# ActiveVisionLab/nope-nerf

Hardware: AMD Instinct MI355X
Metric: training rays/sec (higher is better)
Workload: dtype f32; 1 GPU; BASELINE configs[1]: 1024 rays/GPU x 192 samples, D=256, fp32 via three fp16 MFMA terms per product (fwd, dgrad, wgrad 4x4 + encoding tiles); fp32_products=split2, adam_arithmetic=single, rays_per_gpu=1024, total_rays=1024, n_samples=192, hidden=256, parallelism=dp1 (ray-sharded, one flat all-reduce)

## Files before the change

### nope-nerf_amd/csrc/nnr_api.cpp

```cpp
#include <hip/hip_runtime.h>

#include <algorithm>
#include <cmath>
#include <cstdint>
#include <cstdlib>
#include <cstring>
#include <array>
#include <vector>

#include "../../include/nnr.h"
#include "nnr_device.h"
#include "nnr_kernels.h"
#include "nnr_layout.h"

using namespace nnr;

namespace {

thread_local int g_last_hip = 0;

int hip_fail(hipError_t e) {
    g_last_hip = (int)e;
    return NNR_E_HIP;
}

bool aligned16(const void* p) { return (reinterpret_cast<uintptr_t>(p) & 15u) == 0; }

int check_cfg(const nnr_cfg* c) {
    if (!c || c->n_rays <= 0 || c->n_samples <= 0) return NNR_E_BADCFG;
    if (c->hidden != 128 && c->hidden != 256) return NNR_E_UNSUPPORTED;
    if ((c->flags & NNR_F_TRAIN) && c->n_samples > 1024) return NNR_E_UNSUPPORTED;
    return NNR_OK;
}

WsLayout ws_layout(const nnr_cfg* c) {
    WsLayout w;
    w.S = (int64_t)c->n_rays * c->n_samples;
    w.S_pad = (w.S + kBlockSamples - 1) / kBlockSamples * kBlockSamples;
    w.D = c->hidden;
    w.train = (c->flags & NNR_F_TRAIN) != 0;
    w.bf16 = w.train && (c->flags & NNR_F_BF16) != 0;
    w.tile32 = w.train && (c->flags & (NNR_F_BF16 | NNR_F_SPLIT3)) == NNR_F_SPLIT3;
    return w;
}

int64_t plane(const WsLayout& w, int id) {
    int pitch;
    return w.plane(id, &pitch);
}

size_t packed_floats(int D, int mode) {
    if (mode == 3) return D == 256 ? (size_t)Layout<256, 3>::packed_floats : (size_t)Layout<128, 3>::packed_floats;
    if (mode == 2) return D == 256 ? (size_t)Layout<256, 2>::packed_floats : (size_t)Layout<128, 2>::packed_floats;
    if (mode == 1) return D == 256 ? (size_t)Layout<256, 1>::packed_floats : (size_t)Layout<128, 1>::packed_floats;
    return D == 256 ? (size_t)Layout<256>::packed_floats : (size_t)Layout<128>::packed_floats;
}
bool is_bf16(const nnr_cfg* c) { return (c->flags & NNR_F_BF16) != 0; }
bool is_split3(const nnr_cfg* c) { return (c->flags & (NNR_F_BF16 | NNR_F_SPLIT3)) == NNR_F_SPLIT3; }
bool is_split2(const nnr_cfg* c) { return is_split3(c) && (c->flags & NNR_F_SPLIT2) != 0; }
int weight_mode(const nnr_cfg* c) { return is_bf16(c) ? 1 : (is_split2(c) ? 3 : (is_split3(c) ? 2 : 0)); }

int chunks_per_ray(const nnr_cfg* c) {
    static const bool off = std::getenv("NNR_FLAT_GRID") != nullptr;
    const int unit = is_bf16(c) ? kBf16Tiles * kChunk : kChunk;
    const int waves = is_bf16(c) ? kBf16Waves : kWavesPerBlock;
    return (!off && c->n_samples % unit == 0 && c->n_rays % waves == 0) ? c->n_samples / unit : 0;
}

struct Unit {
    WgradJob j;
    int group;
};

std::vector<Unit> wgrad_units(int D) {
    std::vector<Unit> u;
    const int nb = D / 128;
    int group = 0;
    auto add = [&](int layer, int MI, int NI, int dpl, int dcol, int dvalid, int xpl, int xcol, int xvalid, int row0, int wcol0,
                   int rows_real, int cols_real, int ldw, int bias) {
        Unit x{};
        x.j = WgradJob{layer, MI, NI, dpl, dcol, dvalid, xpl, xcol, xvalid, row0, wcol0, rows_real, cols_real, ldw, 0, 0, bias, 0, -1, 0};
        x.group = group;
        u.push_back(x);
    };
    auto dxd = [&](int layer, int dpl, int xpl, int ldw, int cols_real) {
        for (int a = 0; a < nb; ++a)
            for (int b = 0; b < nb; ++b)
                add(layer, 4, 4, dpl, 128 * a, D - 128 * a, xpl, 128 * b, D - 128 * b, 128 * a, 128 * b, D, cols_real, ldw,
                    nb == 2 ? 2 + b : 1);
        ++group;
// ... 118 lines not shown
    const int64_t group_cost = 4 * 16 * 1000;
    const int64_t group_equiv = std::max<int64_t>(1, (cost_a + cost_b + group_cost / 2) / group_cost);
    const int n_blocks = (int)std::max<int64_t>(2, std::min<int64_t>(max_blocks, granules * group_equiv / kMinGranulesPerBlock));
    int nb_b = (int)((cost_b * n_blocks + (cost_a + cost_b) / 2) / (cost_a + cost_b));
    nb_b = groups.empty() ? n_blocks : std::max(1, std::min(n_blocks - 1, nb_b));
    const int nb_a = n_blocks - nb_b;

    std::vector<std::vector<WgradJob>> per_wave((size_t)n_blocks * 4);
    auto emit = [&](int wave, int unit, int64_t g0, int64_t g1) {
        if (g1 <= g0) return;
        WgradJob j = units[unit].j;
        j.k0 = (int32_t)(g0 * kGranule);
        j.k1 = (int32_t)(g1 * kGranule);
        j.split = unit;
        per_wave[wave].push_back(j);
    };
    const int64_t tape_a = granules * (int64_t)groups.size();
    for (int b = 0; b < nb_a; ++b) {
        const int64_t a0 = tape_a * b / nb_a, a1 = tape_a * (b + 1) / nb_a;
        for (int64_t g = a0 / granules; g <= (a1 - 1) / granules && a1 > a0; ++g) {
            const int64_t lo = std::max(a0, g * granules) - g * granules, hi = std::min(a1, (g + 1) * granules) - g * granules;
            for (int t = 0; t < 4; ++t) emit(4 * b + t, groups[g][t], lo, hi);
        }
    }
    static const bool coop = std::getenv("NNR_WGRAD_NO_COOP") == nullptr;
    if (split && coop)
        for (int wv = 0; wv < 4 * nb_a; ++wv)
            for (auto& j : per_wave[wv]) j.reserved = 1;
    if (!bundles.empty()) {
        int64_t tape = 0;
        for (int64_t cb : bundle_cost) tape += cb * granules;
        int64_t off = 0;
        for (size_t i = 0; i < bundles.size(); ++i) {
            const int64_t cb = bundle_cost[i], end = off + cb * granules;
            auto to_granule = [&](int64_t x) { return std::min(granules, std::max<int64_t>(0, (x - off + cb / 2) / cb)); };
            for (int b = 0; b < nb_b; ++b) {
                const int64_t c0 = tape * b / nb_b, c1 = tape * (b + 1) / nb_b;
                if (c1 <= off || c0 >= end) continue;
                const int64_t g0 = c0 <= off ? 0 : to_granule(c0), g1 = c1 >= end ? granules : to_granule(c1);
                for (int t = 0; t < 4; ++t)
                    for (int u : bundles[i][t]) emit(4 * (nb_a + b) + t, u, g0, g1);
            }
            off = end;
        }
    }
    const int nw_b = nb_b * 4;
    const int64_t tape_b = cost_b * granules;
    std::vector<int64_t> cuts((size_t)nw_b + 1);
    for (int v = 0; v <= nw_b; ++v) cuts[v] = tape_b * v / nw_b;
    int64_t off = 0;
    for (int u : bundles.empty() ? small : std::vector<int>{}) {
        const int64_t cu = weight(units[u].j), end = off + cu * granules;
        auto to_granule = [&](int64_t x) { return std::min(granules, std::max<int64_t>(0, (x - off + cu / 2) / cu)); };
        for (int v = 0; v < nw_b; ++v) {
            if (cuts[v + 1] <= off || cuts[v] >= end) continue;
            const int64_t g0 = cuts[v] <= off ? 0 : to_granule(cuts[v]);
            const int64_t g1 = cuts[v + 1] >= end ? granules : to_granule(cuts[v + 1]);
            emit(4 * nb_a + v, u, g0, g1);
        }
        off = end;
    }
    for (auto& v : per_wave)
        for (auto& j : v)
            if (is_enc2(j)) j.reserved = 2;
    Plan p;
    p.wave_first.push_back(0);
    for (auto& v : per_wave) {
        for (auto& j : v) p.jobs.push_back(j);
        p.wave_first.push_back((int32_t)p.jobs.size());
    }
    std::vector<std::vector<int>> by_tile(units.size());
    for (size_t i = 0; i < p.jobs.size(); ++i) by_tile[p.jobs[i].split].push_back((int)i);
    for (auto& v : by_tile) {
        std::sort(v.begin(), v.end(), [&](int x, int y) { return p.jobs[x].k0 < p.jobs[y].k0; });
        for (size_t s = 0; s < v.size(); ++s) {
            p.jobs[v[s]].split = (int32_t)s;
            p.jobs[v[s]].next_split = s + 1 < v.size() ? v[s + 1] : -1;
        }
        if (!v.empty()) p.heads.push_back(v[0]);
    }
    return p;
}

constexpr int32_t kPlanMagic = 0x4e4e5235;
size_t plan_bytes(const Plan& p) { return p.jobs.size() * sizeof(WgradJob) + (p.wave_first.size() + 1 + p.heads.size() + 4) * sizeof(int32_t); }

struct BUnit {
    int d_plane, d_g0, d_groups, x_plane, x_g0, x_groups, MT, NT, WR, WC, bias;
    int x2_plane = -1, x2_groups = 0;
};
struct BPlan {
    std::vector<WgradJobB> jobs;
    std::vector<int32_t> block_first;
    std::vector<WgradOutB> outs;
};

void bf16_units(int D, std::vector<BUnit>& units, std::vector<WgradOutB>& outs) {
    const int G = D / 16, Gh = D / 32;
    const bool big = D == 256;
    static const bool no_merge = std::getenv("NNR_WGRAD_NO_MERGE") != nullptr;
    const bool merge = big && !no_merge;
    auto out = [&](int unit, int layer, int d_row, int n_rows, int w_row, int x_col, int n_cols, int w_col, int ldw, int bias) {
        const BUnit& u = units[unit];
        outs.push_back(WgradOutB{unit, layer, d_row, n_rows, w_row, x_col, n_cols, w_col, ldw, bias, -1, u.MT, u.NT, u.WR, u.WC, 0});
    };
    auto dxd = [&](int layer, int dpl, int xpl, int ldw) {
        units.push_back(BUnit{dpl, 0, G, xpl, 0, G, big ? 4 : 2, big ? 4 : 2, 2, 2, 1});
        out((int)units.size() - 1, layer, 0, D, 0, 0, D, 0, ldw, 1);
    };
    auto dxe = [&](int layer, int dpl, int w_col, int ldw, int bias) {
        units.push_back(BUnit{dpl, 0, G, P_XE16, 0, kPosPad / 16, big ? 2 : 1, 2, 4, 1, bias});
        out((int)units.size() - 1, layer, 0, D, 0, 0, kPosReal, w_col, ldw, bias);
    };
    dxe(0, P_DH1 + 0, 0, kPosReal, 1);
    dxd(1, P_DH1 + 1, P_XH1 + 0, D);
    dxd(2, P_DH1 + 2, P_XH1 + 1, D);
    dxd(3, P_DH1 + 3, P_XH1 + 2, D);
    if (merge) {
        units.push_back(BUnit{P_DH1 + 4, 0, G, P_XH1 + 3, 0, G, 4, 5, 2, 2, 1, P_XE16, kPosPad / 16});
        out((int)units.size() - 1, 4, 0, D, 0, 0, D, 0, D + kPosReal, 1);
        out((int)units.size() - 1, 4, 0, D, 0, D, kPosReal, D, D + kPosReal, 0);
    } else {
        dxd(4, P_DH1 + 4, P_XH1 + 3, D + kPosReal);
        dxe(4, P_DH1 + 4, D, D + kPosReal, 0);
    }
    dxd(5, P_DH1 + 5, P_XH1 + 4, D);
    dxd(6, P_DH1 + 6, P_XH1 + 5, D);
    dxd(7, P_DH1 + 7, P_XH1 + 6, D);
    if (merge) {
        units.push_back(BUnit{P_DG, 0, Gh + 1, P_XH1 + 7, 0, G, 5, 3, 1, 3, 1, P_XF16, kDirPad / 16});
        out((int)units.size() - 1, kMergedLayer, 0, D / 2, 0, 0, D, 0, D, 1);
        out((int)units.size() - 1, 8, D / 2 + 3, 1, 0, 0, D, 0, D, 1);
        out((int)units.size() - 1, 10, 0, D / 2, 0, D, kDirReal, D, D + kDirReal, 0);
    } else {
        units.push_back(BUnit{P_DG, 0, Gh + 1, P_XH1 + 7, 0, G, big ? 5 : 3, big ? 2 : 1, 1, 4, 1});
        out((int)units.size() - 1, kMergedLayer, 0, D / 2, 0, 0, D, 0, D, 1);
        out((int)units.size() - 1, 8, D / 2 + 3, 1, 0, 0, D, 0, D, 1);
        units.push_back(BUnit{P_DG, 0, Gh, P_XF16, 0, kDirPad / 16, 1, 1, big ? 4 : 2, 1, 0});
        out((int)units.size() - 1, 10, 0, D / 2, 0, 0, kDirReal, D, D + kDirReal, 0);
    }
    units.push_back(BUnit{P_DG, Gh, 1, P_XG, 0, Gh, 1, 1, 1, big ? 4 : 2, 1});
    out((int)units.size() - 1, 11, 0, 3, 0, 0, D / 2, 0, D / 2, 1);
}

constexpr int64_t kMinTapePerBlock = 16 * 32;

BPlan build_plan_bf16(const nnr_cfg* c) {
    const WsLayout w = ws_layout(c);
    BPlan p;
    std::vector<BUnit> units;
    bf16_units(c->hidden, units, p.outs);
    const int64_t chunks = w.S_pad / 32;
    std::vector<int64_t> cost(units.size()), start(units.size() + 1, 0);
    for (size_t u = 0; u < units.size(); ++u) {
        cost[u] = units[u].d_groups + units[u].x_groups + units[u].x2_groups;
        start[u + 1] = start[u] + cost[u] * chunks;
    }
    const int64_t tape = start[units.size()];
    static const int max_blocks = [] {
        const char* e = std::getenv("NNR_WGRAD_MAX_BLOCKS");
        return e ? std::max(1, std::atoi(e)) : kMaxBlocks;
    }();
    const int n_blocks = (int)std::max<int64_t>(1, std::min<int64_t>(max_blocks, tape / kMinTapePerBlock));
    auto cut_chunk = [&](size_t u, int64_t x) {
        if (x <= start[u]) return (int64_t)0;
        if (x >= start[u + 1]) return chunks;
// ... 129 lines not shown
    int pitch = 0;
    const int64_t o = ws_layout(cfg).plane(pl, &pitch);
    if (pitch_out) *pitch_out = pitch;
    return pl < 0 ? -1 : o;
}

int nnr_ws_plane_layout(const nnr_cfg* cfg, int pl) {
    if (check_cfg(cfg) != NNR_OK) return -1;
    const WsLayout w = ws_layout(cfg);
    int pitch = 0;
    if (pl < 0 || w.plane(pl, &pitch) < 0) return -1;
    if (w.tiled(pl)) return 2;
    if (w.bf16 && ((pl >= P_XH1 && pl < P_XH1 + 8) || pl == P_XG || pl == P_XE16 || pl == P_XF16 || (pl >= P_DH1 && pl < P_DH1 + 8) || pl == P_DG)) return 1;
    return 0;
}

size_t nnr_plan_bytes(const nnr_cfg* cfg) {
    if (check_cfg(cfg) != NNR_OK) return 0;
    if (is_bf16(cfg)) return plan_bytes(build_plan_bf16(cfg));
    return plan_bytes(build_plan(cfg));
}

int nnr_plan_counts(const nnr_cfg* cfg, int32_t* n_jobs, int32_t* n_waves) {
    int rc = check_cfg(cfg);
    if (rc != NNR_OK) return rc;
    if (is_bf16(cfg)) {
        const BPlan p = build_plan_bf16(cfg);
        if (n_jobs) *n_jobs = (int32_t)p.jobs.size();
        if (n_waves) *n_waves = 4 * ((int32_t)p.block_first.size() - 1);
        return NNR_OK;
    }
    const Plan p = build_plan(cfg);
    if (n_jobs) *n_jobs = (int32_t)p.jobs.size();
    if (n_waves) *n_waves = (int32_t)p.wave_first.size() - 1;
    return NNR_OK;
}

int nnr_plan_build(const nnr_cfg* cfg, void* plan_host) {
    int rc = check_cfg(cfg);
    if (rc != NNR_OK) return rc;
    if (!plan_host) return NNR_E_BADCFG;
    if (is_bf16(cfg)) {
        const BPlan p = build_plan_bf16(cfg);
        char* out = static_cast<char*>(plan_host);
        std::memcpy(out, p.jobs.data(), p.jobs.size() * sizeof(WgradJobB));
        out += p.jobs.size() * sizeof(WgradJobB);
        std::memcpy(out, p.block_first.data(), p.block_first.size() * sizeof(int32_t));
        out += p.block_first.size() * sizeof(int32_t);
        std::memcpy(out, p.outs.data(), p.outs.size() * sizeof(WgradOutB));
        return NNR_OK;
    }
    const Plan p = build_plan(cfg);
    std::memcpy(plan_host, p.jobs.data(), p.jobs.size() * sizeof(WgradJob));
    char* tail = static_cast<char*>(plan_host) + p.jobs.size() * sizeof(WgradJob);
    std::memcpy(tail, p.wave_first.data(), p.wave_first.size() * sizeof(int32_t));
    tail += p.wave_first.size() * sizeof(int32_t);
    const int32_t n_heads = (int32_t)p.heads.size();
    std::memcpy(tail, &n_heads, sizeof(int32_t));
    std::memcpy(tail + sizeof(int32_t), p.heads.data(), p.heads.size() * sizeof(int32_t));
    const int32_t trailer[4] = {kPlanMagic, (int32_t)p.jobs.size(), (int32_t)p.wave_first.size() - 1, n_heads};
    std::memcpy(tail + sizeof(int32_t) * (1 + p.heads.size()), trailer, sizeof(trailer));
    return NNR_OK;
}

int nnr_pack_weights(const nnr_cfg* cfg, const nnr_params* p, float* packed, void* stream) {
    int rc = check_cfg(cfg);
    if (rc != NNR_OK) return rc;
    if (!p || !packed) return NNR_E_BADCFG;
    if (!aligned16(packed)) return NNR_E_ALIGN;
    PackArgs a;
    for (int i = 0; i < 12; ++i) {
        if (!p->weight[i] || !p->bias[i]) return NNR_E_BADCFG;
        a.w[i] = p->weight[i];
        a.b[i] = p->bias[i];
    }
    a.packed = packed;
    hipError_t e = launch_pack(cfg->hidden, a, weight_mode(cfg), (hipStream_t)stream);
    return e == hipSuccess ? NNR_OK : hip_fail(e);
}

static float* plane_max_of(const nnr_cfg* cfg, float* ws) {
    const WsLayout w = ws_layout(cfg);
    const size_t merged = (size_t)(cfg->hidden / 2) * cfg->hidden + cfg->hidden / 2;
    return ws + (size_t)w.total() + build_plan(cfg).jobs.size() * (size_t)kSlotFloats + merged;
}

static int mlp_fwd_impl(const nnr_cfg* cfg, const float* pts_o, const float* pts_d, const float* view_d, const float* z_lo,
                        const float* z_hi, const float* jitter, const float* packed, float* ws, float* fuse_rgb, float* fuse_dist,
                        void* stream) {
    int rc = check_cfg(cfg);
    if (rc != NNR_OK) return rc;
    if (!pts_o || !pts_d || !view_d || !z_lo || !z_hi || !packed || !ws) return NNR_E_BADCFG;
    if (!aligned16(packed) || !aligned16(ws)) return NNR_E_ALIGN;
    const WsLayout w = ws_layout(cfg);
    MlpFwdArgs a{};
    a.pts_o = pts_o; a.pts_d = pts_d; a.view_d = view_d; a.z_lo = z_lo; a.z_hi = z_hi; a.jitter = jitter;
    a.packed = packed;
    a.ws_out4 = ws + plane(w, P_OUT4);
    a.ws_z = ws + plane(w, P_Z);
    if (w.train) {
        a.ws_xe = ws + plane(w, P_XE);
        a.ws_xh = ws + plane(w, P_XH1);
        a.ws_xf = ws + plane(w, P_XF);
        a.ws_xg = ws + plane(w, P_XG);
        if (w.bf16) {
            a.ws_xe16 = ws + plane(w, P_XE16);
            a.ws_xf16 = ws + plane(w, P_XF16);
            a.ws_pts = ws + plane(w, P_DPTS);
            a.ws_view = ws + plane(w, P_DVIEW);
        }
        a.ws_mask = reinterpret_cast<uint32_t*>(ws + plane(w, P_MASK));
        if (is_split2(cfg)) {
            a.plane_max = plane_max_of(cfg, ws);
            hipError_t em = hipMemsetAsync(a.plane_max, 0, kPlaneMaxFloats * sizeof(float), (hipStream_t)stream);
            if (em != hipSuccess) return hip_fail(em);
        }
    }
    a.S = w.S; a.S_pad = w.S_pad; a.N = cfg->n_samples;
    a.chunks_per_ray = chunks_per_ray(cfg);
    a.fuse_rgb = fuse_rgb; a.fuse_dist = fuse_dist; a.flags = cfg->flags;
    hipError_t e = is_bf16(cfg) ? launch_mlp_fwd_bf16(cfg->hidden, a, w.train, (hipStream_t)stream)
                                : launch_mlp_fwd(cfg->hidden, a, w.train, (hipStream_t)stream, weight_mode(cfg));
    return e == hipSuccess ? NNR_OK : hip_fail(e);
}

int nnr_mlp_fwd(const nnr_cfg* cfg, const float* pts_o, const float* pts_d, const float* view_d, const float* z_lo,
                const float* z_hi, const float* jitter, const float* packed, float* ws, void* stream) {
    return mlp_fwd_impl(cfg, pts_o, pts_d, view_d, z_lo, z_hi, jitter, packed, ws, nullptr, nullptr, stream);
}

int nnr_composite_fwd(const nnr_cfg* cfg, float* rgb, float* dist, float* opt_alpha, float* opt_z, float* ws, void* stream) {
    int rc = check_cfg(cfg);
    if (rc != NNR_OK) return rc;
    if (!rgb || !dist || !ws) return NNR_E_BADCFG;
    const WsLayout w = ws_layout(cfg);
    CompositeArgs a{};
    a.ws_out4 = ws + plane(w, P_OUT4);
    a.ws_z = ws + plane(w, P_Z);
    a.rgb = rgb; a.dist = dist; a.opt_alpha = opt_alpha; a.opt_z = opt_z;
    a.R = cfg->n_rays; a.N = cfg->n_samples; a.flags = cfg->flags;
    hipError_t e = launch_composite_fwd(a, (hipStream_t)stream);
    return e == hipSuccess ? NNR_OK : hip_fail(e);
}

int nnr_render_fwd(const nnr_cfg* cfg, const float* pts_o, const float* pts_d, const float* view_d, const float* z_lo,
                   const float* z_hi, const float* jitter, const float* packed, float* rgb, float* dist, float* opt_alpha,
                   float* opt_z, float* ws, void* stream) {
    static const bool no_fuse = std::getenv("NNR_NO_FUSED_COMPOSITE") != nullptr;
    if (cfg && !(cfg->flags & NNR_F_TRAIN) && !opt_alpha && !opt_z && rgb && dist && !no_fuse && chunks_per_ray(cfg) > 0)
        return mlp_fwd_impl(cfg, pts_o, pts_d, view_d, z_lo, z_hi, jitter, packed, ws, rgb, dist, stream);
    int rc = nnr_mlp_fwd(cfg, pts_o, pts_d, view_d, z_lo, z_hi, jitter, packed, ws, stream);
    if (rc != NNR_OK) return rc;
    return nnr_composite_fwd(cfg, rgb, dist, opt_alpha, opt_z, ws, stream);
}

int nnr_ray_march(const nnr_cfg* cfg, const float* ray_o, const float* ray_d, float radius, const float* t_table, int32_t n_secant,
                  const float* packed, float* state, float* d_out, void* stream) {
    if (!cfg || cfg->n_rays <= 0 || n_secant < 0) return NNR_E_BADCFG;
    if (cfg->hidden != 128 && cfg->hidden != 256) return NNR_E_UNSUPPORTED;
    if (cfg->n_samples < 2 || cfg->n_samples > 1024 || (cfg->flags & (NNR_F_TRAIN | NNR_F_WHITE_BG)) || !is_split2(cfg)) return NNR_E_UNSUPPORTED;
    if (!ray_o || !ray_d || !t_table || !packed || !state || !d_out) return NNR_E_BADCFG;
    if (!aligned16(packed) || !aligned16(state)) return NNR_E_ALIGN;
    MarchArgs a{};
    a.ray_o = ray_o; a.ray_d = ray_d; a.t = t_table; a.packed = packed; a.state = state;
    a.radius = radius; a.R = cfg->n_rays; a.n_steps = cfg->n_samples;
    a.flags = cfg->flags & (NNR_F_RELU_SIGMA | NNR_F_DIST_ALPHA);
    const hipStream_t st = (hipStream_t)stream;
// ... 59 lines not shown

int nnr_composite_bwd(const nnr_cfg* cfg, const float* d_rgb, const float* d_dist, float* ws, void* stream) {
    int rc = check_cfg(cfg);
    if (rc != NNR_OK) return rc;
    if (!(cfg->flags & NNR_F_TRAIN) || !d_rgb || !d_dist || !ws) return NNR_E_BADCFG;
    const WsLayout w = ws_layout(cfg);
    CompositeArgs a{};
    a.ws_out4 = ws + plane(w, P_OUT4);
    a.ws_z = ws + plane(w, P_Z);
    a.ws_dout4 = ws + plane(w, P_DOUT4);
    a.d_rgb = d_rgb; a.d_dist = d_dist;
    a.R = cfg->n_rays; a.N = cfg->n_samples; a.flags = cfg->flags;
    hipError_t e = launch_composite_bwd(a, (hipStream_t)stream);
    return e == hipSuccess ? NNR_OK : hip_fail(e);
}

int nnr_mlp_dgrad(const nnr_cfg* cfg, const float* packed, float* ws, void* stream) {
    int rc = check_cfg(cfg);
    if (rc != NNR_OK) return rc;
    if (!(cfg->flags & NNR_F_TRAIN) || !packed || !ws) return NNR_E_BADCFG;
    if (!aligned16(packed) || !aligned16(ws)) return NNR_E_ALIGN;
    const WsLayout w = ws_layout(cfg);
    MlpDgradArgs a{};
    a.packed = packed;
    a.ws_dout4 = ws + plane(w, P_DOUT4);
    a.ws_xe = ws + plane(w, P_XE);
    a.ws_xf = ws + plane(w, P_XF);
    a.ws_mask = reinterpret_cast<const uint32_t*>(ws + plane(w, P_MASK));
    a.ws_dh = ws + plane(w, P_DH1);
    a.ws_dg = ws + plane(w, P_DG);
    a.ws_dpts = ws + plane(w, P_DPTS);
    a.ws_dview = ws + plane(w, P_DVIEW);
    a.plane_max = is_split2(cfg) ? plane_max_of(cfg, ws) : nullptr;
    a.S = w.S; a.S_pad = w.S_pad;
    a.chunks_per_ray = chunks_per_ray(cfg);
    hipError_t e = is_bf16(cfg) ? launch_mlp_dgrad_bf16(cfg->hidden, a, (hipStream_t)stream)
                                : launch_mlp_dgrad(cfg->hidden, a, (hipStream_t)stream, weight_mode(cfg));
    return e == hipSuccess ? NNR_OK : hip_fail(e);
}

int nnr_mlp_wgrad(const nnr_cfg* cfg, const float* packed, const nnr_param_grads* g, const void* plan, float* ws, void* stream) {
    int rc = check_cfg(cfg);
    if (rc != NNR_OK) return rc;
    if (!(cfg->flags & NNR_F_TRAIN) || !packed || !g || !plan || !ws) return NNR_E_BADCFG;
    const WsLayout w = ws_layout(cfg);
    if (w.bf16) {
        WgradBArgs b{};
        for (int i = 0; i < 12; ++i) {
            if (!g->weight[i] || !g->bias[i]) return NNR_E_BADCFG;
            b.gw[i] = g->weight[i];
            b.gb[i] = g->bias[i];
        }
        const BPlan p = build_plan_bf16(cfg);
        b.n_jobs = (int)p.jobs.size();
        b.n_blocks = (int)p.block_first.size() - 1;
        b.n_outs = (int)p.outs.size();
        b.jobs = static_cast<const WgradJobB*>(plan);
        b.block_first = reinterpret_cast<const int32_t*>(b.jobs + b.n_jobs);
        b.outs = reinterpret_cast<const WgradOutB*>(b.block_first + b.n_blocks + 1);
        b.ws = ws;
        b.slots = ws + w.total();
        b.gw[kMergedLayer] = b.slots + (size_t)b.n_jobs * 4 * kSlotBFloats;
        b.gb[kMergedLayer] = b.gw[kMergedLayer] + (size_t)(cfg->hidden / 2) * cfg->hidden;
        b.packed = packed;
        b.D = cfg->hidden;
        hipError_t e = launch_wgrad_bf16(b, (hipStream_t)stream);
        return e == hipSuccess ? NNR_OK : hip_fail(e);
    }
    WgradArgs a{};
    for (int i = 0; i < 12; ++i) {
        if (!g->weight[i] || !g->bias[i]) return NNR_E_BADCFG;
        a.gw[i] = g->weight[i];
        a.gb[i] = g->bias[i];
    }
    a.jobs = static_cast<const WgradJob*>(plan);
    a.ws = ws;
    for (int p = 0; p < 48; ++p) {
        int pitch = 0;
        a.plane_off[p] = w.plane(p, &pitch);
        a.plane_pitch[p] = pitch;
        a.plane_tile[p] = w.tiled(p) ? 1 : 0;
    }
    {
        const Plan p = build_plan(cfg);
        a.n_jobs = (int)p.jobs.size();
        a.n_waves = (int)p.wave_first.size() - 1;
        a.n_heads = (int)p.heads.size();
    }
    a.wave_first = reinterpret_cast<const int32_t*>(a.jobs + a.n_jobs);
    a.heads = a.wave_first + a.n_waves + 2;
    a.slots = ws + w.total();
    a.gw[kMergedLayer] = a.slots + (size_t)a.n_jobs * kSlotFloats;
    a.gb[kMergedLayer] = a.gw[kMergedLayer] + (size_t)(cfg->hidden / 2) * cfg->hidden;
    a.packed = packed;
    a.D = cfg->hidden;
    a.plane_max = is_split2(cfg) ? plane_max_of(cfg, ws) : nullptr;
    a.bf16 = weight_mode(cfg);
    {
        const int D = cfg->hidden;
        const int rows[13] = {D, D, D, D, D, D, D, D, 1, D, D / 2, 3, D / 2};
        for (int l = 0; l < 13; ++l) a.bias_rows[l] = rows[l];
    }
    hipError_t e = launch_wgrad(a, (hipStream_t)stream);
    return e == hipSuccess ? NNR_OK : hip_fail(e);
}

int nnr_ray_reduce(const nnr_cfg* cfg, float* d_pts_o, float* d_pts_d, float* d_view, float* ws, void* stream) {
    int rc = check_cfg(cfg);
    if (rc != NNR_OK) return rc;
    if (!(cfg->flags & NNR_F_TRAIN) || !d_pts_o || !d_pts_d || !d_view || !ws) return NNR_E_BADCFG;
    const WsLayout w = ws_layout(cfg);
    RayReduceArgs a{};
    a.ws_dpts = ws + plane(w, P_DPTS);
    a.ws_dview = ws + plane(w, P_DVIEW);
    a.ws_z = ws + plane(w, P_Z);
    a.d_pts_o = d_pts_o; a.d_pts_d = d_pts_d; a.d_view = d_view;
    a.R = cfg->n_rays; a.N = cfg->n_samples;
    hipError_t e = launch_ray_reduce(a, (hipStream_t)stream);
    return e == hipSuccess ? NNR_OK : hip_fail(e);
}

int nnr_render_bwd(const nnr_cfg* cfg, const float* packed, const float* d_rgb, const float* d_dist,
                   const nnr_param_grads* grads, float* d_pts_o, float* d_pts_d, float* d_view, const void* plan, float* ws,
                   void* stream) {
    int rc = nnr_composite_bwd(cfg, d_rgb, d_dist, ws, stream);
    if (rc != NNR_OK) return rc;
    rc = nnr_mlp_dgrad(cfg, packed, ws, stream);
    if (rc != NNR_OK) return rc;
    rc = nnr_mlp_wgrad(cfg, packed, grads, plan, ws, stream);
    if (rc != NNR_OK) return rc;
    return nnr_ray_reduce(cfg, d_pts_o, d_pts_d, d_view, ws, stream);
}

#define NNR_LAUNCH(expr) do { hipError_t e_ = (expr); return e_ == hipSuccess ? NNR_OK : hip_fail(e_); } while (0)

int nnr_se3_exp_fwd(const float* r_all, const float* t_all, int32_t idx, float* c2w, void* stream) {
    if (!r_all || !t_all || !c2w || idx < 0) return NNR_E_BADCFG;
    NNR_LAUNCH(launch_se3_exp_fwd(r_all, t_all, idx, c2w, (hipStream_t)stream));
}
int nnr_se3_exp_bwd(const float* r_all, int32_t idx, int32_t n_cams, const float* d_c2w, float* d_r_all, float* d_t_all,
                    void* stream) {
    if (!r_all || !d_c2w || !d_r_all || !d_t_all || idx < 0 || idx >= n_cams) return NNR_E_BADCFG;
    NNR_LAUNCH(launch_se3_exp_bwd(r_all, idx, n_cams, d_c2w, d_r_all, d_t_all, (hipStream_t)stream));
}
int nnr_inv4_fwd(const float* a, float* y, int32_t batch, void* stream) {
    if (!a || !y || batch <= 0) return NNR_E_BADCFG;
    NNR_LAUNCH(launch_inv4(a, y, batch, (hipStream_t)stream));
}
int nnr_inv4_bwd(const float* y, const float* d_y, float* d_a, int32_t batch, void* stream) {
    if (!y || !d_y || !d_a || batch <= 0) return NNR_E_BADCFG;
    NNR_LAUNCH(launch_inv4_bwd(y, d_y, d_a, batch, (hipStream_t)stream));
}
int nnr_ray_setup_fwd(const float* pixels, const float* depth, const float* K, const float* W, const float* S, int32_t n_rays,
                      int32_t normalise, int32_t use_dir, float* pts_o, float* dir, float* view, float* ray_norm, float* d_gt,
                      uint8_t* mask, void* stream) {
    if (!pixels || !K || !W || !S || !pts_o || !dir || !view || !ray_norm || !d_gt || !mask || n_rays <= 0) return NNR_E_BADCFG;
    RaySetupArgs a{};
    a.pixels = pixels; a.depth = depth; a.K = K; a.W = W; a.S = S;
    a.pts_o = pts_o; a.dir = dir; a.view = view; a.ray_norm = ray_norm; a.d_gt = d_gt; a.mask = mask;
    a.R = n_rays; a.normalise = normalise; a.use_dir = use_dir;
    NNR_LAUNCH(launch_ray_setup_fwd(a, (hipStream_t)stream));
}
int nnr_ray_setup_bwd(const float* pixels, const float* depth, const float* K, const float* W, const float* S, int32_t n_rays,
                      int32_t normalise, int32_t use_dir, const float* g_pts_o, const float* g_dir, const float* g_view,
                      const float* g_ray_norm, const float* g_d_gt, float* d_depth, float* dK, float* dW, float* dS,
                      float* scratch, void* stream) {
    if (!pixels || !K || !W || !S || !dK || !dW || !dS || !scratch || n_rays <= 0) return NNR_E_BADCFG;
    RaySetupArgs a{};
    a.pixels = pixels; a.depth = depth; a.K = K; a.W = W; a.S = S;
    a.g_o = g_pts_o; a.g_dir = g_dir; a.g_view = g_view; a.g_norm = g_ray_norm; a.g_dgt = g_d_gt;
// ... 218 lines not shown
```

### nope-nerf_amd/csrc/nnr_wgrad.hip

```cpp
#include "nnr_device.h"
#include "nnr_kernels.h"
#include "nnr_split.h"
#include <cstdlib>

namespace nnr {

NNR_TL_DECL(tl_wgrad)
#ifdef NNR_TIMELINE
__device__ unsigned long long tl_wgrad_all[4096];
extern "C" int nnr_timeline_wgrad_all(unsigned long long* host4096) {
    return (int)hipMemcpyFromSymbol(host4096, HIP_SYMBOL(tl_wgrad_all), 4096 * sizeof(unsigned long long));
}
#endif

template <int W>
struct Vec { float v[W]; };

template <int W>
__device__ __forceinline__ Vec<W> load_vec(const float* p) {
    Vec<W> r;
    if constexpr (W == 4) {
        const f32x4 t = *reinterpret_cast<const f32x4*>(p);
        r.v[0] = t[0]; r.v[1] = t[1]; r.v[2] = t[2]; r.v[3] = t[3];
    } else if constexpr (W == 2) {
// ... 845 lines not shown
            NNR_WGRAD_CASE(4, 2)
            NNR_WGRAD_CASE(4, 1)
            NNR_WGRAD_CASE(2, 4)
            NNR_WGRAD_CASE(2, 1)
            NNR_WGRAD_CASE(1, 4)
            NNR_WGRAD_CASE(1, 2)
            default: break;
        }
#undef NNR_WGRAD_CASE
#undef NNR_WGRAD_RUN
    }
#ifdef NNR_TIMELINE
    if (lane == 0 && wslot < 2048) tl_wgrad_all[2 * wslot + 1] = __builtin_amdgcn_s_memtime();
#endif
}

hipError_t launch_wgrad_f16_main(const WgradArgs& a, hipStream_t st);
#ifdef NNR_WGRAD_F16_TU
hipError_t launch_wgrad_f16_main(const WgradArgs& a, hipStream_t st) {
    hipLaunchKernelGGL((wgrad_kernel<true, true>), dim3(a.n_waves / 4), dim3(256), 0, st, a);
    return hipGetLastError();
}
#else
constexpr int kMaxChain = 256;
__global__ __launch_bounds__(256) void wgrad_reduce_kernel(WgradArgs a) {
    const int ji = a.heads[blockIdx.x >> 4];
    const WgradJob jb = a.jobs[ji];
    __shared__ int chain[kMaxChain];
    __shared__ int n_chain;
    if (threadIdx.x == 0) {
        int n = 0, j = ji;
        for (; j >= 0 && n < kMaxChain; j = a.jobs[j].next_split) chain[n++] = j - ji;
        if (j >= 0) __builtin_trap();
        n_chain = n;
    }
    __syncthreads();
    const int n = n_chain;
    const int t = (blockIdx.x & 15) * 256 + threadIdx.x;
    const int pitch = 32 * jb.NI, f4_per_row = 8 * jb.NI;
    const int row = t / f4_per_row, c0 = 4 * (t - row * f4_per_row);
    if (row < 32 * jb.MI && row < jb.d_valid && jb.row0 + row < jb.rows_real) {
        f32x4 sum = {0.f, 0.f, 0.f, 0.f};
        const float* src = a.slots + (int64_t)ji * kSlotFloats + row * pitch + c0;
        int s = 0;
        for (; s + 8 <= n; s += 8) {
            f32x4 v[8];
#pragma unroll
            for (int u = 0; u < 8; ++u) v[u] = *reinterpret_cast<const f32x4*>(src + (int64_t)chain[s + u] * kSlotFloats);
#pragma unroll
            for (int u = 0; u < 8; ++u) sum += v[u];
        }
        for (; s < n; ++s) sum += *reinterpret_cast<const f32x4*>(src + (int64_t)chain[s] * kSlotFloats);
        if (a.plane_max != nullptr && jb.reserved == 2) {
            const float sd = plane_scale(a.plane_max[8 + (jb.d_plane - P_DH1)]), sx = plane_scale(a.plane_max[kPlaneMaxEnc]);
            sum = (sum * (1.f / sd)) * (1.f / sx);
        }
        if (a.plane_max != nullptr && jb.reserved == 1) {
            const float sd = plane_scale(a.plane_max[jb.d_plane == P_DG ? 16 : 8 + (jb.d_plane - P_DH1)]), sx = plane_scale(a.plane_max[jb.x_plane - P_XH1]);
            sum = (sum * (1.f / sd)) * (1.f / sx);
        }
        float* dst = a.gw[jb.layer] + (int64_t)(jb.row0 + row) * jb.ldw + jb.wcol0 + c0;
#pragma unroll
        for (int e = 0; e < 4; ++e)
            if (c0 + e < jb.x_valid && jb.wcol0 + c0 + e < jb.cols_real) dst[e] = sum[e];
    }
    if (jb.bias && (blockIdx.x & 15) == 0 && (int)threadIdx.x < 32 * jb.MI) {
        const int r = threadIdx.x;
        if (r < jb.d_valid && jb.row0 + r < jb.rows_real) {
            float sum = 0.f;
            const float* src = a.slots + (int64_t)ji * kSlotFloats + kSlotTile + r;
            for (int s = 0; s < n; ++s) {
                const float* p = src + (int64_t)chain[s] * kSlotFloats;
                sum += p[0] + p[32 * jb.MI];
            }
            atomicAdd(a.gb[jb.layer] + jb.row0 + r, sum);
        }
    }
}

template <int D, int BF16>
__global__ __launch_bounds__(256) void wgrad_unmerge_kernel(WgradArgs a) {
    using L = Layout<D, BF16>;
    constexpr int Dh = L::Dh, ldg = D + kDirReal;
    const float* Wf = a.packed + L::copy_wf_off;
    const float* Wg1 = a.packed + L::copy_wg_off;
    const float* bf = a.packed + L::copy_bf_off;
    const float* dWm = a.gw[kMergedLayer];
    const float* dbm = a.gb[kMergedLayer];
    const int gid = blockIdx.x * 256 + threadIdx.x;
    if (gid < D * D) {
        const int j = gid / D, k = gid - j * D;
        float acc = 0.f;
#pragma unroll 16
        for (int m = 0; m < Dh; ++m) acc = fmaf(Wg1[m * D + j], dWm[m * D + k], acc);
        a.gw[9][gid] = acc;
    } else if (gid < D * D + Dh * D) {
        const int t = gid - D * D, m = t / D, j = t - m * D;
        float acc = dbm[m] * bf[j];
#pragma unroll 16
        for (int k = 0; k < D; ++k) acc = fmaf(dWm[m * D + k], Wf[j * D + k], acc);
        a.gw[10][m * ldg + j] = acc;
    } else if (gid < D * D + Dh * D + D) {
        const int j = gid - D * D - Dh * D;
        float acc = 0.f;
        for (int m = 0; m < Dh; ++m) acc = fmaf(Wg1[m * D + j], dbm[m], acc);
        a.gb[9][j] = acc;
    } else if (gid < D * D + Dh * D + D + Dh) {
        const int m = gid - D * D - Dh * D - D;
        a.gb[10][m] = dbm[m];
    }
}

hipError_t launch_wgrad(const WgradArgs& a, hipStream_t st) {
    hipError_t e;
    prof_before(PROF_WGRAD, st);
    static const bool split_off = std::getenv("NNR_WGRAD_FP32") != nullptr;
    static const bool f16_off = std::getenv("NNR_WGRAD_BF16_TERMS") != nullptr;
    WgradArgs b = a;
    if (!(a.bf16 == 3 && a.plane_max != nullptr && !split_off && !f16_off)) b.plane_max = nullptr;
    if (b.plane_max != nullptr) (void)launch_wgrad_f16_main(b, st);
    else if (a.bf16 >= 2 && !split_off) hipLaunchKernelGGL(wgrad_kernel<true>, dim3(a.n_waves / 4), dim3(256), 0, st, b);
    else hipLaunchKernelGGL(wgrad_kernel<false>, dim3(a.n_waves / 4), dim3(256), 0, st, b);
    hipLaunchKernelGGL(wgrad_reduce_kernel, dim3(a.n_heads * 16), dim3(256), 0, st, b);
    e = hipGetLastError();
    if (e == hipSuccess) e = launch_wgrad_unmerge(a, st);
    prof_after(PROF_WGRAD, st);
    return e;
}

hipError_t launch_wgrad_unmerge(const WgradArgs& a, hipStream_t st) {
    const int threads = a.D * a.D + (a.D / 2) * a.D + a.D + a.D / 2;
    const dim3 grid((threads + 255) / 256), block(256);
    if (a.D == 256) {
        if (a.bf16 == 3) hipLaunchKernelGGL((wgrad_unmerge_kernel<256, 3>), grid, block, 0, st, a);
        else if (a.bf16 == 2) hipLaunchKernelGGL((wgrad_unmerge_kernel<256, 2>), grid, block, 0, st, a);
        else if (a.bf16 == 1) hipLaunchKernelGGL((wgrad_unmerge_kernel<256, 1>), grid, block, 0, st, a);
        else hipLaunchKernelGGL((wgrad_unmerge_kernel<256, 0>), grid, block, 0, st, a);
    } else {
        if (a.bf16 == 3) hipLaunchKernelGGL((wgrad_unmerge_kernel<128, 3>), grid, block, 0, st, a);
        else if (a.bf16 == 2) hipLaunchKernelGGL((wgrad_unmerge_kernel<128, 2>), grid, block, 0, st, a);
        else if (a.bf16 == 1) hipLaunchKernelGGL((wgrad_unmerge_kernel<128, 1>), grid, block, 0, st, a);
        else hipLaunchKernelGGL((wgrad_unmerge_kernel<128, 0>), grid, block, 0, st, a);
    }
    return hipGetLastError();
}

#endif

}
```

Baseline: 452,400 rays/s.

## Tile the wgrad unmerge GEMMs through shared memory and cache plan counts

The unmerge kernel's two small matrix products now run as 16x16 output tiles per block. Operand panels are staged in shared memory, so each thread no longer streams strided rows from global memory. Separately, the host path stops rebuilding the whole wgrad plan each step just to read job, wave and head counts; it memoises them in a mutex-protected map keyed by hidden size, padded sample count and flags. The tiled kernel adds syncthreads and up to about 33 KB of LDS per block for D=256, and the cache relies on the key fully determining the plan.

```diff
diff --git a/nope-nerf_amd/csrc/nnr_api.cpp b/nope-nerf_amd/csrc/nnr_api.cpp
--- a/nope-nerf_amd/csrc/nnr_api.cpp
+++ b/nope-nerf_amd/csrc/nnr_api.cpp
@@ -6,6 +6,9 @@
 #include <cstdlib>
 #include <cstring>
 #include <array>
+#include <map>
+#include <mutex>
+#include <tuple>
 #include <vector>
 
 #include "../../include/nnr.h"
@@ -290,6 +293,28 @@
     return p;
 }
 
+struct PlanCounts {
+    int32_t n_jobs, n_waves, n_heads;
+};
+PlanCounts plan_counts_uncached(const nnr_cfg* c) {
+    const Plan p = build_plan(c);
+    return PlanCounts{(int32_t)p.jobs.size(), (int32_t)p.wave_first.size() - 1, (int32_t)p.heads.size()};
+}
+PlanCounts plan_counts(const nnr_cfg* c) {
+    static std::mutex mu;
+    static std::map<std::tuple<int32_t, int64_t, uint32_t>, PlanCounts> known;
+    const auto key = std::make_tuple((int32_t)c->hidden, (int64_t)ws_layout(c).S_pad, (uint32_t)c->flags);
+    {
+        std::lock_guard<std::mutex> lock(mu);
+        const auto it = known.find(key);
+        if (it != known.end()) return it->second;
+    }
+    const PlanCounts pc = plan_counts_uncached(c);
+    std::lock_guard<std::mutex> lock(mu);
+    known.emplace(key, pc);
+    return pc;
+}
+
 constexpr int32_t kPlanMagic = 0x4e4e5235;
 size_t plan_bytes(const Plan& p) { return p.jobs.size() * sizeof(WgradJob) + (p.wave_first.size() + 1 + p.heads.size() + 4) * sizeof(int32_t); }
 
@@ -585,7 +610,7 @@
 static float* plane_max_of(const nnr_cfg* cfg, float* ws) {
     const WsLayout w = ws_layout(cfg);
     const size_t merged = (size_t)(cfg->hidden / 2) * cfg->hidden + cfg->hidden / 2;
-    return ws + (size_t)w.total() + build_plan(cfg).jobs.size() * (size_t)kSlotFloats + merged;
+    return ws + (size_t)w.total() + (size_t)plan_counts(cfg).n_jobs * (size_t)kSlotFloats + merged;
 }
 
 static int mlp_fwd_impl(const nnr_cfg* cfg, const float* pts_o, const float* pts_d, const float* view_d, const float* z_lo,
@@ -811,10 +836,10 @@
         a.plane_tile[p] = w.tiled(p) ? 1 : 0;
     }
     {
-        const Plan p = build_plan(cfg);
-        a.n_jobs = (int)p.jobs.size();
-        a.n_waves = (int)p.wave_first.size() - 1;
-        a.n_heads = (int)p.heads.size();
+        const PlanCounts pc = plan_counts(cfg);
+        a.n_jobs = pc.n_jobs;
+        a.n_waves = pc.n_waves;
+        a.n_heads = pc.n_heads;
     }
     a.wave_first = reinterpret_cast<const int32_t*>(a.jobs + a.n_jobs);
     a.heads = a.wave_first + a.n_waves + 2;
diff --git a/nope-nerf_amd/csrc/nnr_wgrad.hip b/nope-nerf_amd/csrc/nnr_wgrad.hip
--- a/nope-nerf_amd/csrc/nnr_wgrad.hip
+++ b/nope-nerf_amd/csrc/nnr_wgrad.hip
@@ -951,31 +951,53 @@
 __global__ __launch_bounds__(256) void wgrad_unmerge_kernel(WgradArgs a) {
     using L = Layout<D, BF16>;
     constexpr int Dh = L::Dh, ldg = D + kDirReal;
+    constexpr int kTilesF = (D / 16) * (D / 16), kTilesG = (Dh / 16) * (D / 16);
     const float* Wf = a.packed + L::copy_wf_off;
     const float* Wg1 = a.packed + L::copy_wg_off;
     const float* bf = a.packed + L::copy_bf_off;
     const float* dWm = a.gw[kMergedLayer];
     const float* dbm = a.gb[kMergedLayer];
-    const int gid = blockIdx.x * 256 + threadIdx.x;
-    if (gid < D * D) {
-        const int j = gid / D, k = gid - j * D;
+    __shared__ float lds[2 * 16 * (D + 1)];
+    const int hi = threadIdx.x >> 4, lo = threadIdx.x & 15;
+    if ((int)blockIdx.x < kTilesF) {
+        const int j0 = 16 * ((int)blockIdx.x / (D / 16)), k0 = 16 * ((int)blockIdx.x % (D / 16));
+        float (*wg_s)[16] = reinterpret_cast<float (*)[16]>(lds);
+        float (*dw_s)[16] = reinterpret_cast<float (*)[16]>(lds + Dh * 16);
+        for (int i = threadIdx.x; i < Dh * 16; i += 256) {
+            wg_s[i / 16][i % 16] = Wg1[(i / 16) * D + j0 + i % 16];
+            dw_s[i / 16][i % 16] = dWm[(i / 16) * D + k0 + i % 16];
+        }
+        __syncthreads();
         float acc = 0.f;
 #pragma unroll 16
-        for (int m = 0; m < Dh; ++m) acc = fmaf(Wg1[m * D + j], dWm[m * D + k], acc);
-        a.gw[9][gid] = acc;
-    } else if (gid < D * D + Dh * D) {
-        const int t = gid - D * D, m = t / D, j = t - m * D;
+        for (int m = 0; m < Dh; ++m) acc = fmaf(wg_s[m][hi], dw_s[m][lo], acc);
+        a.gw[9][(j0 + hi) * D + k0 + lo] = acc;
+        return;
+    }
+    if ((int)blockIdx.x < kTilesF + kTilesG) {
+        const int t = (int)blockIdx.x - kTilesF, m0 = 16 * (t / (D / 16)), j0 = 16 * (t % (D / 16));
+        float (*dw_s)[D + 1] = reinterpret_cast<float (*)[D + 1]>(lds);
+        float (*wf_s)[D + 1] = reinterpret_cast<float (*)[D + 1]>(lds + 16 * (D + 1));
+        for (int i = threadIdx.x; i < 16 * D; i += 256) {
+            dw_s[i / D][i % D] = dWm[(m0 + i / D) * D + i % D];
+            wf_s[i / D][i % D] = Wf[(j0 + i / D) * D + i % D];
+        }
+        __syncthreads();
+        const int m = m0 + hi, j = j0 + lo;
         float acc = dbm[m] * bf[j];
 #pragma unroll 16
-        for (int k = 0; k < D; ++k) acc = fmaf(dWm[m * D + k], Wf[j * D + k], acc);
+        for (int k = 0; k < D; ++k) acc = fmaf(dw_s[hi][k], wf_s[lo][k], acc);
         a.gw[10][m * ldg + j] = acc;
-    } else if (gid < D * D + Dh * D + D) {
-        const int j = gid - D * D - Dh * D;
+        return;
+    }
+    const int gid = ((int)blockIdx.x - kTilesF - kTilesG) * 256 + threadIdx.x;
+    if (gid < D) {
+        const int j = gid;
         float acc = 0.f;
         for (int m = 0; m < Dh; ++m) acc = fmaf(Wg1[m * D + j], dbm[m], acc);
         a.gb[9][j] = acc;
-    } else if (gid < D * D + Dh * D + D + Dh) {
-        const int m = gid - D * D - Dh * D - D;
+    } else if (gid < D + Dh) {
+        const int m = gid - D;
         a.gb[10][m] = dbm[m];
     }
 }
@@ -998,8 +1020,8 @@
 }
 
 hipError_t launch_wgrad_unmerge(const WgradArgs& a, hipStream_t st) {
-    const int threads = a.D * a.D + (a.D / 2) * a.D + a.D + a.D / 2;
-    const dim3 grid((threads + 255) / 256), block(256);
+    const int tiles = (a.D / 16) * (a.D / 16) + (a.D / 32) * (a.D / 16);
+    const dim3 grid(tiles + (a.D + a.D / 2 + 255) / 256), block(256);
     if (a.D == 256) {
         if (a.bf16 == 3) hipLaunchKernelGGL((wgrad_unmerge_kernel<256, 3>), grid, block, 0, st, a);
         else if (a.bf16 == 2) hipLaunchKernelGGL((wgrad_unmerge_kernel<256, 2>), grid, block, 0, st, a);
```

After: 452,600 rays/s, median of 2. No clear change (+0.0%).
